# lucasjinreal/yolov7_d2

Measured on AMD Instinct MI355X. Metric: images/sec training, YOLOX-s 640x640 bs=16/GPU, higher is better.
Workload: dtype bf16; 1 GPU; YOLOX-s CSPDarknet+PAFPN 640x640 bs=16/GPU: fwd + SimOTA loss + bwd + grad all-reduce + SGD(momentum) step, uint8 image batch + labels resident in HBM; global_batch=16, parallelism=dp1, hipgraph=True

## Files before the change

### yolov7_d2_amd/csrc/conv3x3_ws.h

```cpp
#pragma once
#include "common.h"
#include "conv_bn.h"

#define W3_MAX_JOBS 8
#define W3_TW 16
template <int S, int TH>
struct W3Geo {
  static constexpr int HH = S == 1 ? TH + 2 : 2 * TH + 1;
  static constexpr int HW = S == 1 ? W3_TW + 2 : 2 * W3_TW + 1;
  static constexpr int HPIX = HH * HW;
  static constexpr int HROWS = (HPIX + 63) / 64 * 64;
  static constexpr int tap(int dy, int dx) { return S == 1 ? dy * HW + dx : dy * HW + (dx & 1) * (W3_TW + 1) + (dx >> 1); }
};

struct W3Job {
  const __bf16* x;
  const u32x4* w;
  __bf16* y;
  double* stats;
  int ldx, ldy, N, H, W, tilesY, tilesX, ntiles;
  int blk0, nblk;
  int wld, nslots, sld, pad_;
  int tw[9];
  int inH;
  int inW, xfw;
  const BnXf* xf;
};
struct W3K {
  int njobs, dbg;
  W3Job j[W3_MAX_JOBS];
};
struct W3Launch {
  int K, MODE, grid, lds, S, XF;
  W3K k;
};

#define W3_VMCNT(n) asm volatile("s_waitcnt vmcnt(%0)" ::"n"(n) : "memory")

static __device__ uint4 g_w3_zero_page[4];

__device__ __forceinline__ void w3_glds16(const void* g, unsigned lds_off) {
  asm volatile("s_mov_b32 m0, %1\n\ts_nop 0\n\tglobal_load_lds_dwordx4 %0, off" ::"v"(g), "s"(lds_off) : "memory");
}

template <int K, int WM, int WN, int G, int MODE, int S = 1, int TH = 8, int XF = 0>
__global__ __launch_bounds__(WM* WN * 64, (K == 128 || (S == 2 && K == 64)) ? 1 : 2) void w3_kernel(const W3K p) {
  static_assert(!XF || MODE == 1, "the input transform comes with the forward (statistics) mode");
  constexpr int NW = WM * WN, KC8 = K / 8, KS = K / 16;
  using Geo = W3Geo<S, TH>;
  constexpr int W3_TH = TH, W3_HW = Geo::HW, W3_HPIX = Geo::HPIX, W3_HROWS = Geo::HROWS;
  static_assert(WN * G * 32 == W3_TH * W3_TW, "pixel tile");
  constexpr int PLANE = W3_HROWS * 16;
  constexpr int NQ = (W3_HROWS / 64) * KC8;
  constexpr int D = NQ / NW;
  static_assert(NQ % NW == 0 && D >= 1, "DMA split");
  constexpr int XB = KC8 * PLANE;
  static_assert((KC8 - 1) * PLANE + Geo::tap(2, 2) * 16 < 65536, "ds_read immediate");
  constexpr int NS = 9 * KS, NTS = NS / 3;
  constexpr int NST = 2 * G;
  constexpr int DST = 2 * (D - 1) < NTS ? 2 : 1, SST = 2 * NST + NST / 2 <= NTS ? 2 : 1;
  static_assert(DST * (D - 1) < NTS && SST * NST + (MODE == 2 ? NST / 2 : 0) <= NTS, "the memory operations of a tile fit its main loop");

  extern __shared__ __attribute__((aligned(16))) char smem[];
  const unsigned lds0 = (unsigned)(uintptr_t)(__attribute__((address_space(3))) char*)smem;
  const int tid = threadIdx.x, lane = tid & 63;
  const int wave = __builtin_amdgcn_readfirstlane(tid >> 6);
  const int wm = wave / WN, wn = wave % WN;
  const int l31 = lane & 31, h = lane >> 5;

  int ji = 0;
  while (ji + 1 < p.njobs && (int)blockIdx.x >= p.j[ji + 1].blk0) ++ji;
  ji = __builtin_amdgcn_readfirstlane(ji);
  const W3Job& jb = p.j[ji];
  const int b = (int)blockIdx.x - jb.blk0, nb = jb.nblk;
  const int nt = (jb.ntiles - b + nb - 1) / nb;
  constexpr bool STATS = MODE == 1;
  const int H = jb.H, Wd = jb.W, tilesX = jb.tilesX, tpi = jb.tilesY * jb.tilesX;
  const int inH = S == 1 ? jb.H : jb.inH, inW = S == 1 ? jb.W : jb.inW;
  const int ldxb = jb.ldx * 2, ldyb = jb.ldy * 2;
  const char* const xbase = (const char*)jb.x;
  char* const ybase = (char*)jb.y;
  const char* zpage = (const char*)g_w3_zero_page;
  asm volatile("" : "+s"(zpage));
  float* const s_sc = (float*)(smem + 2 * (K / 8) * Geo::HROWS * 16 + 256 * 32 * 4);
  float* const s_sh = s_sc + K;
  int xf_act = 0, xf_ldab = 0;
  char* xf_a = nullptr;
  if constexpr (XF) {
    const BnXf* const xf = jb.xf;
    bnx_tables(xf, s_sc, s_sh, NW * 64, jb.xfw != 0 && b == 0);
    xf_act = xf->bn.act;
    xf_ldab = xf->bn.lda * 2;
    xf_a = jb.xfw ? (char*)xf->bn.a : nullptr;
  }

  bf16x8 a[9][KS];
  {
    const u32x4* wb = jb.w + wm * 32 + l31;
#pragma unroll
    for (int t = 0; t < 9; ++t) {
      const int slab = jb.tw[t] * KC8;
#pragma unroll
      for (int ks = 0; ks < KS; ++ks) a[t][ks] = __builtin_bit_cast(bf16x8, wb[(size_t)(slab + ks * 2 + h) * jb.wld]);
    }
  }

  struct Org { int img, ty0, tx0; };
  auto tile_origin = [&](int i) {
    const int t = b + i * nb;
    Org o;
    o.img = t / tpi;
    const int rem = t - o.img * tpi, tyq = rem / tilesX;
    o.ty0 = tyq * W3_TH;
    o.tx0 = (rem - tyq * tilesX) * W3_TW;
    return o;
  };
  auto issue_x1 = [&](const Org& o, int buf, int d) {
    const int iy0 = S * o.ty0 - 1, ix0 = S * o.tx0 - 1;
    const char* xt = xbase + ((size_t)o.img * inH * inW + (ptrdiff_t)iy0 * inW + ix0) * (ptrdiff_t)ldxb;
    const int q = wave * D + d;
    const int pb = q / KC8, k8 = q % KC8;
    const int pix = pb * 64 + lane;
    const int hy = S == 1 ? (int)(((unsigned)pix * 3641u) >> 16) : (int)(((unsigned)pix * 1986u) >> 16);
    const int hp = pix - hy * W3_HW;
    const int hx = S == 1 ? hp : (hp <= W3_TW ? 2 * hp : 2 * (hp - (W3_TW + 1)) + 1);
    const bool v = (pix < W3_HPIX) & ((unsigned)(iy0 + hy) < (unsigned)inH) & ((unsigned)(ix0 + hx) < (unsigned)inW);
    const char* g = v ? xt + (unsigned)((hy * inW + hx) * ldxb + k8 * 16) : zpage;
    w3_glds16(g, lds0 + buf * XB + k8 * PLANE + pb * 1024);
  };

  int lg, lidx;
  {
    const int l = l31;
    lg = ((l >= 4) & (l < 12)) | ((l >= 16) & (l < 20)) | (l >= 28);
    lidx = l - (l < 4 ? 0 : l < 12 ? 4 : l < 20 ? 8 : l < 28 ? 12 : 16);
  }
  unsigned bbase[G];
#pragma unroll
  for (int g = 0; g < G; ++g) bbase[g] = (unsigned)(h * PLANE + (S * ((wn * G + g) * 2 + lg) * W3_HW + lidx) * 16);
  auto out_ptr = [&](const Org& o, int g) -> char* {
    const int py = o.ty0 + (wn * G + g) * 2 + lg, px = o.tx0 + lidx;
    char* q = ybase + (((size_t)o.img * H + py) * Wd + px) * (size_t)ldyb + wm * 64 + h * 16;
    return ((py < H) & (px < Wd)) ? q : nullptr;
  };

  constexpr bool SREG = (K == 32 && S == 1) || (K == 64 && S == 2);
  float* const sacc = (float*)(smem + 2 * XB) + tid * 4;
  constexpr int SAS = NW * 64 * 4;
  float s1[16], s2[16];
  if constexpr (STATS) {
    if constexpr (SREG) {
#pragma unroll
      for (int r = 0; r < 16; ++r) s1[r] = s2[r] = 0.f;
    } else {
#pragma unroll
      for (int q = 0; q < 8; ++q) *(f32x4*)(sacc + q * SAS) = f32x4{0.f, 0.f, 0.f, 0.f};
    }
  }

  Org oc = tile_origin(0), op = oc;
#pragma unroll
  for (int d = 0; d < D; ++d) issue_x1(oc, 0, d);

  u32x4 pk[NST];
#pragma unroll
  for (int q = 0; q < NST; ++q) pk[q] = u32x4{0u, 0u, 0u, 0u};
  for (int i = 0; i < nt; ++i) {
    W3_VMCNT(0);
    if constexpr (XF) {
      if (i == 0) __syncthreads();
      const int iy0 = S * oc.ty0 - 1, ix0 = S * oc.tx0 - 1;
      char* const Xw = smem + (i & 1) * XB;
      char* const at = xf_a + ((size_t)oc.img * inH * inW + (ptrdiff_t)iy0 * inW + ix0) * (ptrdiff_t)xf_ldab;
#pragma unroll 2
      for (int d = 0; d < D; ++d) {
        const int q = wave * D + d;
        const int pb = q / KC8, k8 = q % KC8;
        const int pix = pb * 64 + lane;
        const int hy = S == 1 ? (int)(((unsigned)pix * 3641u) >> 16) : (int)(((unsigned)pix * 1986u) >> 16);
        const int hp = pix - hy * W3_HW;
        const int hx = S == 1 ? hp : (hp <= W3_TW ? 2 * hp : 2 * (hp - (W3_TW + 1)) + 1);
        const bool v = (pix < W3_HPIX) & ((unsigned)(iy0 + hy) < (unsigned)inH) & ((unsigned)(ix0 + hx) < (unsigned)inW);
        const u32x4 o = bnx_apply_lds(Xw + k8 * PLANE + pb * 1024 + lane * 16, s_sc, s_sh, k8, xf_act, v);
        const bool inner = v & (hy >= 1) & (hy <= S * W3_TH) & (hx >= 1) & (hx <= S * W3_TW);
        if (xf_a && inner) *(u32x4*)(at + (unsigned)((hy * inW + hx) * xf_ldab + k8 * 16)) = o;
      }
      asm volatile("s_waitcnt lgkmcnt(0)" ::: "memory");
    }
    __builtin_amdgcn_s_barrier();
    const bool more = (i + 1 < nt) & !(p.dbg & 2);
    const bool prev = i > 0;
    const Org on = tile_origin(i + 1 < nt ? i + 1 : i);
    const char* Xs = smem + (i & 1) * XB;
    u32x4 old[NST];

    f32x16 acc[G];
#pragma unroll
    for (int g = 0; g < G; ++g)
#pragma unroll
      for (int r = 0; r < 16; ++r) acc[g][r] = 0.f;
    auto ldb = [&](int step, bf16x8(&dst)[G]) {
      const int t9 = step / KS, ks = step % KS, dy = t9 / 3, dx = t9 % 3;
#pragma unroll
      for (int g = 0; g < G; ++g)
        dst[g] = __builtin_bit_cast(bf16x8, *(const u32x4*)(Xs + bbase[g] + (2 * ks * PLANE + Geo::tap(dy, dx) * 16)));
    };
    bf16x8 bf[3][G];
    ldb(0, bf[0]);
    ldb(1, bf[1]);
    if (!(p.dbg & 4))
#pragma unroll
    for (int ts = 0; ts < NTS; ++ts) {
      if (ts % DST == 0 && ts / DST < D) {
        if (more) issue_x1(on, (i + 1) & 1, ts / DST);
      }
      if (ts % SST == SST - 1 && ts / SST < NST) {
        char* q = prev ? out_ptr(op, (ts / SST) / 2) : nullptr;
        if (q) *(u32x4*)(q + ((ts / SST) % 2) * 32) = pk[ts / SST];
      }
      if constexpr (MODE == 2) {
        if (ts >= SST * NST && ts < SST * NST + NST / 2) {
#pragma unroll
          for (int l = 2 * (ts - SST * NST); l < 2 * (ts - SST * NST) + 2; ++l) {
            char* q = out_ptr(oc, l / 2);
            old[l] = u32x4{0u, 0u, 0u, 0u};
            if (q) {
              if (l % 2 == 0) asm volatile("global_load_dwordx4 %0, %1, off" : "+v"(old[l]) : "v"(q) : "memory");
              else asm volatile("global_load_dwordx4 %0, %1, off offset:32" : "+v"(old[l]) : "v"(q) : "memory");
            }
          }
        }
      }
#pragma unroll
      for (int r = 0; r < 3; ++r) {
        const int st = 3 * ts + r;
        __builtin_amdgcn_sched_barrier(0);
        if (st + 2 < NS) ldb(st + 2, bf[(r + 2) % 3]);
#pragma unroll
        for (int g = 0; g < G; ++g)
          acc[g] = __builtin_amdgcn_mfma_f32_32x32x16_bf16(a[st / KS][st % KS], bf[r][g], acc[g], 0, 0, 0);
#pragma unroll
        for (int g = 0; g < G; ++g) {
          __builtin_amdgcn_sched_group_barrier(0x008, 1, 0);
          __builtin_amdgcn_sched_group_barrier(0x100, 1, 0);
          __builtin_amdgcn_sched_group_barrier(0x002, 2, 0);
        }
      }
      __builtin_amdgcn_sched_barrier(0);
    }

    if constexpr (MODE == 2) {
      if constexpr (NST == 2)
        asm volatile("s_waitcnt vmcnt(0)" : "+v"(old[0]), "+v"(old[1])::"memory");
      else if constexpr (NST == 4)
        asm volatile("s_waitcnt vmcnt(0)" : "+v"(old[0]), "+v"(old[1]), "+v"(old[2]), "+v"(old[3])::"memory");
      else
        asm volatile("s_waitcnt vmcnt(0)"
                     : "+v"(old[0]), "+v"(old[1]), "+v"(old[2]), "+v"(old[3]), "+v"(old[4]), "+v"(old[5]), "+v"(old[6]), "+v"(old[7])::"memory");
    }
    if constexpr (STATS && !SREG) {
#pragma unroll
      for (int q = 0; q < 4; ++q) {
        const f32x4 u = *(const f32x4*)(sacc + q * SAS), w = *(const f32x4*)(sacc + (4 + q) * SAS);
#pragma unroll
        for (int e = 0; e < 4; ++e) { s1[4 * q + e] = u[e]; s2[4 * q + e] = w[e]; }
      }
    }
#pragma unroll
    for (int g = 0; g < G; ++g) {
      bool pvg = true;
      if constexpr (STATS) pvg = out_ptr(oc, g) != nullptr;
      unsigned pw[8];
#pragma unroll
      for (int q = 0; q < 4; ++q) {
        bf16x4 o;
#pragma unroll
        for (int e = 0; e < 4; ++e) o[e] = (__bf16)acc[g][4 * q + e];
        if constexpr (STATS) {
#pragma unroll
          for (int e = 0; e < 4; ++e) {
            const float f = pvg ? (float)o[e] : 0.f;
            s1[4 * q + e] += f;
            s2[4 * q + e] = __builtin_fmaf(f, f, s2[4 * q + e]);
          }
        }
        const u32x2 u = __builtin_bit_cast(u32x2, o);
        pw[2 * q] = u[0];
        pw[2 * q + 1] = u[1];
      }
#pragma unroll
      for (int pr = 0; pr < 2; ++pr) {
        const int q0 = 2 * pr, q1 = 2 * pr + 1;
        const auto w0 = __builtin_amdgcn_permlane32_swap(pw[2 * q0], pw[2 * q1], false, false);
        const auto w1 = __builtin_amdgcn_permlane32_swap(pw[2 * q0 + 1], pw[2 * q1 + 1], false, false);
        u32x4 v = {w0[0], w1[0], w0[1], w1[1]};
        if constexpr (MODE == 2) {
          const bf16x8 nv = __builtin_bit_cast(bf16x8, v), ov = __builtin_bit_cast(bf16x8, old[g * 2 + pr]);
          bf16x8 rv;
#pragma unroll
          for (int e = 0; e < 8; ++e) rv[e] = (__bf16)((float)nv[e] + (float)ov[e]);
          v = __builtin_bit_cast(u32x4, rv);
        }
        pk[g * 2 + pr] = v;
      }
    }
    if constexpr (STATS && !SREG) {
#pragma unroll
      for (int q = 0; q < 4; ++q) {
        *(f32x4*)(sacc + q * SAS) = f32x4{s1[4 * q], s1[4 * q + 1], s1[4 * q + 2], s1[4 * q + 3]};
        *(f32x4*)(sacc + (4 + q) * SAS) = f32x4{s2[4 * q], s2[4 * q + 1], s2[4 * q + 2], s2[4 * q + 3]};
      }
    }
    op = oc;
    oc = on;
  }
#pragma unroll
  for (int q = 0; q < NST; ++q) {
    char* o = out_ptr(op, q / 2);
    if (o) *(u32x4*)(o + (q % 2) * 32) = pk[q];
  }

  if constexpr (STATS) {
    if constexpr (!SREG) {
#pragma unroll
      for (int q = 0; q < 4; ++q) {
        const f32x4 u = *(const f32x4*)(sacc + q * SAS), w = *(const f32x4*)(sacc + (4 + q) * SAS);
#pragma unroll
        for (int e = 0; e < 4; ++e) { s1[4 * q + e] = u[e]; s2[4 * q + e] = w[e]; }
      }
    }
    cbn_block_stats<WM, WN>(s1, s2, (float*)smem, wave, lane, (p.dbg & 1) != 0, [&](const int c) {
      return jb.stats + (size_t)((int)blockIdx.x % jb.nslots) * jb.sld + c * 2;
    });
  }
}

template <int K, int WM, int WN, int G, int MODE, int S = 1, int TH = 8, int XF = 0>
static int w3_launch_one(const W3Launch& l, hipStream_t s) {
  auto fn = w3_kernel<K, WM, WN, G, MODE, S, TH, XF>;
  static bool attr_done = false;
  if (!attr_done) {
    hipFuncSetAttribute((const void*)fn, hipFuncAttributeMaxDynamicSharedMemorySize, 160 * 1024);
    attr_done = true;
  }
  hipLaunchKernelGGL(fn, dim3((unsigned)l.grid), dim3(WM * WN * 64), (size_t)l.lds, s, l.k);
  MI_CHECK_LAUNCH("conv3x3_ws");
  return MI_OK;
}
constexpr int w3_tile_h(int S, int K) { return S == 1 ? 8 : (K == 128 ? 2 : 4); }
constexpr int w3_block_cout(int S, int K) { return S == 1 ? K : (K == 32 ? 64 : 128); }
template <int MODE, int XF = 0>
static int w3_launch_mode(const W3Launch& l, hipStream_t s) {
  if (l.S == 2) {
    if constexpr (MODE == 1 || MODE == 0) {
      switch (l.K) {
        case 128: return w3_launch_one<128, 4, 1, 1, MODE, 2, 2, XF>(l, s);
        case 64: return w3_launch_one<64, 4, 1, 2, MODE, 2, 4, XF>(l, s);
        case 32: return w3_launch_one<32, 2, 2, 1, MODE, 2, 4, XF>(l, s);
      }
    }
    MI_FAIL(MI_EINVAL, "conv3x3_ws: stride 2 with K %d / mode %d", l.K, MODE);
  }
  switch (l.K) {
    case 128: return w3_launch_one<128, 4, 1, 4, MODE, 1, 8, XF>(l, s);
    case 64: return w3_launch_one<64, 2, 2, 2, MODE, 1, 8, XF>(l, s);
    case 32: return w3_launch_one<32, 1, 4, 1, MODE, 1, 8, XF>(l, s);
  }
  MI_FAIL(MI_EINVAL, "conv3x3_ws: K %d", l.K);
}
```

### yolov7_d2_amd/csrc/conv3x3_ws.hip

```cpp
#include <stdlib.h>
#include <string.h>
#include "common.h"
#include "conv3x3_ws.h"

int w3_launch_mode0(const W3Launch& l, hipStream_t s);
int w3_launch_mode1(const W3Launch& l, hipStream_t s);
int w3_launch_mode1x(const W3Launch& l, hipStream_t s);
int w3_launch_mode2(const W3Launch& l, hipStream_t s);

static int w3_cus() {
  static int cus = 0;
  if (!cus) {
    int dev = 0;
    hipDeviceProp_t pr;
    if (hipGetDevice(&dev) == hipSuccess && hipGetDeviceProperties(&pr, dev) == hipSuccess) cus = pr.multiProcessorCount;
    if (cus <= 0) cus = 256;
  }
  return cus;
}

static bool w3_desc_ok(const mi_conv_desc* d, int* tw) {
  const int K = d->K8 * 8;
  if (d->ntaps != 9 || (d->in_stride != 1 && d->in_stride != 2) || d->out_stride != 1 || d->out_oy || d->out_ox) return false;
  if (d->gridH != d->outH || d->gridW != d->outW) return false;
  if (d->flags & ~MI_CONV_ACCUM) return false;
  if (d->bias) return false;
  if (!(K == 32 || K == 64 || K == 128) || d->Cout != d->CoutPad) return false;
  if (d->in_stride == 1) {
    if (d->outH != d->H || d->outW != d->W || d->Cout != K) return false;
  } else {
    const char* s2 = getenv("MI_CONV_WS_S2");
    if ((s2 && atoi(s2) == 0) || (d->flags & MI_CONV_ACCUM)) return false;
    if (d->outH != (d->H - 1) / 2 + 1 || d->outW != (d->W - 1) / 2 + 1) return false;
    const int bc = w3_block_cout(2, K);
    if (d->Cout % bc || d->Cout / bc > W3_MAX_JOBS) return false;
  }
  if (d->ldx % 8 || d->ldy % 8 || ((uintptr_t)d->x & 15) || ((uintptr_t)d->y & 15) || ((uintptr_t)d->w & 15)) return false;
  if (d->y_nstride && (long long)d->y_nstride != (long long)d->outH * d->outW * d->ldy) return false;
  if ((long long)d->H * d->W * d->ldx * 2 >= (1LL << 31)) return false;
  if ((d->flags & MI_CONV_ACCUM) && d->stats_acc) return false;
  int seen = 0;
  for (int t = 0; t < 9; ++t) {
    const int dy = d->tap_dy[t], dx = d->tap_dx[t];
    if (dy < -1 || dy > 1 || dx < -1 || dx > 1) return false;
    const int pos = (dy + 1) * 3 + dx + 1;
    if (seen & (1 << pos)) return false;
    seen |= 1 << pos;
    tw[pos] = d->tap_w[t];
  }
  return seen == 0x1ff;
}

static bool w3_fill(const mi_conv_desc* ds, int n, W3Launch* l) {
  if (n < 1 || n > W3_MAX_JOBS) return false;
  memset(l, 0, sizeof(*l));
  const int K = ds[0].K8 * 8, S = ds[0].in_stride;
  const int mode = (ds[0].flags & MI_CONV_ACCUM) ? 2 : (ds[0].stats_acc ? 1 : 0);
  const bool xf = ds[0].xf != nullptr;
  if (xf && mode != 1) return false;
  const int TH = w3_tile_h(S, K);
  const int hrows = ((S == 1 ? (TH + 2) * (W3_TW + 2) : (2 * TH + 1) * (2 * W3_TW + 1)) + 63) / 64 * 64;
  const int lds = 2 * (K / 8) * hrows * 16 + (mode == 1 ? 256 * 32 * 4 : 0) + (xf ? 2 * K * 4 : 0);
  long long total = 0;
  int nj = 0;
  for (int j = 0; j < n; ++j) {
    const mi_conv_desc& d = ds[j];
    int tw[9];
    if (!w3_desc_ok(&d, tw) || d.K8 * 8 != K || d.in_stride != S) return false;
    if ((d.flags & MI_CONV_ACCUM) != (ds[0].flags & MI_CONV_ACCUM) || (d.stats_acc != nullptr) != (ds[0].stats_acc != nullptr)) return false;
    if ((d.xf != nullptr) != xf || (xf && (d.xf_C != K || ((uintptr_t)d.xf & 7)))) return false;
    const int bc = w3_block_cout(S, K);
    for (int c0 = 0; c0 < d.Cout; c0 += bc, ++nj) {
      if (nj >= W3_MAX_JOBS) return false;
      W3Job& jb = l->k.j[nj];
      memcpy(jb.tw, tw, sizeof(tw));
      jb.x = (const __bf16*)d.x; jb.w = (const u32x4*)d.w + c0; jb.y = (__bf16*)d.y + c0;
      jb.stats = d.stats_acc ? d.stats_acc + (size_t)c0 * 2 : nullptr;
      jb.ldx = d.ldx; jb.ldy = d.ldy; jb.N = d.N; jb.H = d.outH; jb.W = d.outW; jb.inH = d.H; jb.inW = d.W;
      jb.tilesY = mi_cdiv(d.outH, TH); jb.tilesX = mi_cdiv(d.outW, W3_TW);
      jb.ntiles = d.N * jb.tilesY * jb.tilesX;
      jb.wld = d.CoutPad;
      jb.nslots = (d.stats_slots >= 1 && d.stats_slots <= MI_BN_SLOTS) ? d.stats_slots : MI_BN_SLOTS;
      jb.sld = d.CoutPad * 2;
      total += jb.ntiles;
      jb.xf = (const BnXf*)d.xf;
      jb.xfw = (xf && d.xf_write && c0 == 0) ? 1 : 0;
    }
  }
  n = nj;
  int per_cu = K == 128 ? 1 : (K == 64 ? 2 : 4);
  if (S == 2) per_cu = (160 * 1024) / lds >= 2 && K != 128 ? 2 : 1;
  long long cap = (long long)w3_cus() * per_cu;
  if (cap > total) cap = total;
  int used = 0;
  for (int j = 0; j < n; ++j) {
    W3Job& jb = l->k.j[j];
    long long nb = (cap * jb.ntiles) / total;
    if (nb < 1) nb = 1;
    if (nb > jb.ntiles) nb = jb.ntiles;
    jb.nblk = (int)nb;
    used += jb.nblk;
  }
  while (used < cap) {
    int best = -1;
    double br = 0;
    for (int j = 0; j < n; ++j) {
      const W3Job& jb = l->k.j[j];
      const double r = (double)jb.ntiles / jb.nblk;
      if (jb.nblk < jb.ntiles && r > br) { br = r; best = j; }
    }
    if (best < 0) break;
    l->k.j[best].nblk++;
    used++;
  }
  int blk = 0;
  for (int j = 0; j < n; ++j) {
    l->k.j[j].blk0 = blk;
    blk += l->k.j[j].nblk;
  }
  l->k.njobs = n;
  l->k.dbg = (getenv("MI_DEBUG_NOATOM") ? atoi(getenv("MI_DEBUG_NOATOM")) & 1 : 0) | (getenv("MI_W3_DBG") ? atoi(getenv("MI_W3_DBG")) & 6 : 0);
  l->K = K;
  l->S = S;
  l->MODE = mode;
  l->XF = xf ? 1 : 0;
  l->grid = blk;
  l->lds = lds;
  return true;
}

static int w3_run(const W3Launch& l, hipStream_t s) {
  switch (l.MODE) {
    case 0: return w3_launch_mode0(l, s);
    case 1: return l.XF ? w3_launch_mode1x(l, s) : w3_launch_mode1(l, s);
    default: return w3_launch_mode2(l, s);
  }
}

static bool w3_enabled() {
  const char* e = getenv("MI_CONV_WS");
  return !e || atoi(e) != 0;
}

bool w3_try_launch(const mi_conv_desc* ds, int n, hipStream_t s, int* rc) {
  if (!w3_enabled()) return false;
  W3Launch l;
  if (!w3_fill(ds, n, &l)) return false;
  *rc = w3_run(l, s);
  return true;
}
bool w3_try_plan(const mi_conv_desc* ds, int n, W3Launch* l) { return w3_enabled() && w3_fill(ds, n, l); }
int w3_run_planned(const W3Launch* l, hipStream_t s) { return w3_run(*l, s); }

extern "C" int mi_conv3x3_ws(const mi_conv_desc* descs, int n, mi_stream_t st) {
  MI_REQUIRE(descs && n >= 1, "conv3x3_ws: null");
  W3Launch l;
  MI_REQUIRE(w3_fill(descs, n, &l),
             "conv3x3_ws: needs 1..%d bf16 3x3 stride-1 convs with K == Cout in {32, 64, 128} (all the same K), no bias, "
             "all plain / all with stats_acc / all MI_CONV_ACCUM", W3_MAX_JOBS);
  return w3_run(l, (hipStream_t)st);
}
```

Measured before the change: 3179 images/sec.

## Use buffer-resource loads/stores with OOB masking and incremental tile stepping in 3x3 conv

Replaces global_load_lds with zero-page redirection by buffer_load ... lds, using a buffer resource whose out-of-range offsets return zero. Output stores and MODE-2 reloads also go through raw buffer ops with an out-of-bounds sentinel instead of per-store pointer checks. Per-tile index math is reduced by precomputing halo pixel offsets once and advancing tile coordinates incrementally instead of dividing on every tile. It also adds an optional compile-time timeline probe and a new guard that output size fits in 31 bits.

```diff
diff --git a/yolov7_d2_amd/csrc/conv3x3_ws.h b/yolov7_d2_amd/csrc/conv3x3_ws.h
--- a/yolov7_d2_amd/csrc/conv3x3_ws.h
+++ b/yolov7_d2_amd/csrc/conv3x3_ws.h
@@ -29,6 +29,9 @@
 struct W3K {
   int njobs, dbg;
   W3Job j[W3_MAX_JOBS];
+#ifdef MI_W3_TIMELINE
+  unsigned long long* tl;
+#endif
 };
 struct W3Launch {
   int K, MODE, grid, lds, S, XF;
@@ -37,11 +40,43 @@
 
 #define W3_VMCNT(n) asm volatile("s_waitcnt vmcnt(%0)" ::"n"(n) : "memory")
 
-static __device__ uint4 g_w3_zero_page[4];
-
-__device__ __forceinline__ void w3_glds16(const void* g, unsigned lds_off) {
-  asm volatile("s_mov_b32 m0, %1\n\ts_nop 0\n\tglobal_load_lds_dwordx4 %0, off" ::"v"(g), "s"(lds_off) : "memory");
-}
+#define W3_OOB 0x80000000u
+
+__device__ __forceinline__ __amdgpu_buffer_rsrc_t w3_rsrc(const char* base, unsigned bytes) {
+  return __builtin_amdgcn_make_buffer_rsrc((void*)base, 0, (int)bytes, 0x00020000);
+}
+__device__ __forceinline__ void w3_blds16(__amdgpu_buffer_rsrc_t r, unsigned voff, unsigned soff, unsigned lds_off) {
+  asm volatile("s_mov_b32 m0, %3\n\ts_nop 3\n\tbuffer_load_dwordx4 %0, %1, %2 offen lds" ::"v"(voff), "s"(r), "s"(soff), "s"(lds_off) : "memory");
+}
+
+constexpr int w3_dma_blocks(int D, int KC8, int NW) {
+  int m = 1;
+  for (int w = 0; w < NW; ++w) {
+    const int n = (w * D + D - 1) / KC8 - (w * D) / KC8 + 1;
+    m = n > m ? n : m;
+  }
+  return m;
+}
+
+#ifdef MI_W3_TIMELINE
+#define W3_TL_POINTS 12
+#define W3_TL_BLOCKS 1024
+#define W3_TL(k)                                                                                              \
+  do {                                                                                                        \
+    __builtin_amdgcn_sched_barrier(0);                                                                        \
+    if (wave == 0 && blockIdx.x < W3_TL_BLOCKS) {                                                             \
+      unsigned long long tr_, tc_;                                                                            \
+      asm volatile("s_memrealtime %0\n\ts_memtime %1\n\ts_waitcnt lgkmcnt(0)" : "=s"(tr_), "=s"(tc_)::"memory"); \
+      if (lane == 0) {                                                                                        \
+        p.tl[((size_t)blockIdx.x * W3_TL_POINTS + (k)) * 2] = tr_;                                            \
+        p.tl[((size_t)blockIdx.x * W3_TL_POINTS + (k)) * 2 + 1] = tc_;                                        \
+      }                                                                                                       \
+    }                                                                                                         \
+    __builtin_amdgcn_sched_barrier(0);                                                                        \
+  } while (0)
+#else
+#define W3_TL(k) do { } while (0)
+#endif
 
 template <int K, int WM, int WN, int G, int MODE, int S = 1, int TH = 8, int XF = 0>
 __global__ __launch_bounds__(WM* WN * 64, (K == 128 || (S == 2 && K == 64)) ? 1 : 2) void w3_kernel(const W3K p) {
@@ -75,13 +110,13 @@
   const int b = (int)blockIdx.x - jb.blk0, nb = jb.nblk;
   const int nt = (jb.ntiles - b + nb - 1) / nb;
   constexpr bool STATS = MODE == 1;
-  const int H = jb.H, Wd = jb.W, tilesX = jb.tilesX, tpi = jb.tilesY * jb.tilesX;
+  const int H = jb.H, Wd = jb.W, tilesX = jb.tilesX, tilesY = jb.tilesY, tpi = jb.tilesY * jb.tilesX;
   const int inH = S == 1 ? jb.H : jb.inH, inW = S == 1 ? jb.W : jb.inW;
   const int ldxb = jb.ldx * 2, ldyb = jb.ldy * 2;
   const char* const xbase = (const char*)jb.x;
   char* const ybase = (char*)jb.y;
-  const char* zpage = (const char*)g_w3_zero_page;
-  asm volatile("" : "+s"(zpage));
+  const unsigned imgxb = (unsigned)(inH * inW * ldxb), imgyb = (unsigned)(H * Wd * ldyb);
+  W3_TL(0);
   float* const s_sc = (float*)(smem + 2 * (K / 8) * Geo::HROWS * 16 + 256 * 32 * 4);
   float* const s_sh = s_sc + K;
   int xf_act = 0, xf_ldab = 0;
@@ -105,28 +140,63 @@
     }
   }
 
-  struct Org { int img, ty0, tx0; };
-  auto tile_origin = [&](int i) {
-    const int t = b + i * nb;
-    Org o;
-    o.img = t / tpi;
-    const int rem = t - o.img * tpi, tyq = rem / tilesX;
-    o.ty0 = tyq * W3_TH;
-    o.tx0 = (rem - tyq * tilesX) * W3_TW;
+  struct Org { int img, ty, tx; };
+  int s_img, s_ty, s_tx;
+  Org oc;
+  {
+    s_img = nb / tpi;
+    const int r1 = nb - s_img * tpi;
+    s_ty = r1 / tilesX;
+    s_tx = r1 - s_ty * tilesX;
+    oc.img = b / tpi;
+    const int r0 = b - oc.img * tpi;
+    oc.ty = r0 / tilesX;
+    oc.tx = r0 - oc.ty * tilesX;
+  }
+  auto tile_next = [&](Org o) {
+    o.tx += s_tx;
+    const int cx = o.tx >= tilesX;
+    o.tx -= cx ? tilesX : 0;
+    o.ty += s_ty + cx;
+    const int cy = o.ty >= tilesY;
+    o.ty -= cy ? tilesY : 0;
+    o.img += s_img + cy;
     return o;
   };
-  auto issue_x1 = [&](const Org& o, int buf, int d) {
-    const int iy0 = S * o.ty0 - 1, ix0 = S * o.tx0 - 1;
-    const char* xt = xbase + ((size_t)o.img * inH * inW + (ptrdiff_t)iy0 * inW + ix0) * (ptrdiff_t)ldxb;
-    const int q = wave * D + d;
-    const int pb = q / KC8, k8 = q % KC8;
-    const int pix = pb * 64 + lane;
+  constexpr int NPB = w3_dma_blocks(D, KC8, NW);
+  static_assert(NPB <= 2, "sel");
+  const int pb0 = (wave * D) / KC8;
+  unsigned hpix[NPB], hoff[NPB];
+#pragma unroll
+  for (int j = 0; j < NPB; ++j) {
+    const int pix = (pb0 + j) * 64 + lane;
     const int hy = S == 1 ? (int)(((unsigned)pix * 3641u) >> 16) : (int)(((unsigned)pix * 1986u) >> 16);
     const int hp = pix - hy * W3_HW;
     const int hx = S == 1 ? hp : (hp <= W3_TW ? 2 * hp : 2 * (hp - (W3_TW + 1)) + 1);
-    const bool v = (pix < W3_HPIX) & ((unsigned)(iy0 + hy) < (unsigned)inH) & ((unsigned)(ix0 + hx) < (unsigned)inW);
-    const char* g = v ? xt + (unsigned)((hy * inW + hx) * ldxb + k8 * 16) : zpage;
-    w3_glds16(g, lds0 + buf * XB + k8 * PLANE + pb * 1024);
+    const bool in = pix < W3_HPIX;
+    hpix[j] = in ? (unsigned)(hy << 8 | hx) : 0u;
+    hoff[j] = in ? (unsigned)((hy * inW + hx) * ldxb) : W3_OOB;
+  }
+  auto sel = [&](const unsigned(&a)[NPB], int j) {
+    return NPB > 1 && j >= 1 ? a[NPB - 1] : a[0];
+  };
+  struct XT { const char* img; unsigned v[NPB]; };
+  auto x_tile = [&](const Org& o) {
+    const int iy0 = S * o.ty * W3_TH - 1, ix0 = S * o.tx * W3_TW - 1;
+    const unsigned tb = (unsigned)((iy0 * inW + ix0) * ldxb);
+    XT t;
+    t.img = xbase + (size_t)o.img * imgxb;
+#pragma unroll
+    for (int j = 0; j < NPB; ++j) {
+      const bool v = ((unsigned)(iy0 + (int)(hpix[j] >> 8)) < (unsigned)inH) & ((unsigned)(ix0 + (int)(hpix[j] & 255u)) < (unsigned)inW);
+      t.v[j] = v ? tb + hoff[j] : W3_OOB;
+    }
+    return t;
+  };
+  auto issue_x1 = [&](const XT& t, int buf, int d) {
+    const int q = wave * D + d;
+    const int pb = q / KC8, k8 = q % KC8;
+    w3_blds16(w3_rsrc(t.img, imgxb), sel(t.v, pb - pb0), (unsigned)(k8 * 16), lds0 + buf * XB + k8 * PLANE + pb * 1024);
   };
 
   int lg, lidx;
@@ -138,11 +208,18 @@
   unsigned bbase[G];
 #pragma unroll
   for (int g = 0; g < G; ++g) bbase[g] = (unsigned)(h * PLANE + (S * ((wn * G + g) * 2 + lg) * W3_HW + lidx) * 16);
-  auto out_ptr = [&](const Org& o, int g) -> char* {
-    const int py = o.ty0 + (wn * G + g) * 2 + lg, px = o.tx0 + lidx;
-    char* q = ybase + (((size_t)o.img * H + py) * Wd + px) * (size_t)ldyb + wm * 64 + h * 16;
-    return ((py < H) & (px < Wd)) ? q : nullptr;
+  const unsigned yoff0 = (unsigned)((((wn * G) * 2 + lg) * Wd + lidx) * ldyb + wm * 64 + h * 16), ystep = (unsigned)(2 * Wd * ldyb);
+  struct YT { char* img; unsigned v; int rows; };
+  auto y_tile = [&](const Org& o) {
+    const int ty0 = o.ty * W3_TH, tx0 = o.tx * W3_TW;
+    YT t;
+    t.img = ybase + (size_t)o.img * imgyb;
+    t.v = lidx < Wd - tx0 ? (unsigned)((ty0 * Wd + tx0) * ldyb) + yoff0 : W3_OOB;
+    t.rows = H - ty0 - wn * G * 2;
+    return t;
   };
+  auto y_valid = [&](const YT& t, int g) { return (lg < t.rows - 2 * g) & (t.v != W3_OOB); };
+  auto y_off = [&](const YT& t, int g) { return lg < t.rows - 2 * g ? t.v + g * ystep : W3_OOB; };
 
   constexpr bool SREG = (K == 32 && S == 1) || (K == 64 && S == 2);
   float* const sacc = (float*)(smem + 2 * XB) + tid * 4;
@@ -158,9 +235,17 @@
     }
   }
 
-  Org oc = tile_origin(0), op = oc;
-#pragma unroll
-  for (int d = 0; d < D; ++d) issue_x1(oc, 0, d);
+#ifdef MI_W3_TIMELINE
+  W3_VMCNT(0);
+#endif
+  W3_TL(1);
+  {
+    const XT x0 = x_tile(oc);
+#pragma unroll
+    for (int d = 0; d < D; ++d) issue_x1(x0, 0, d);
+  }
+  YT yc = y_tile(oc), yp = yc;
+  yp.v = W3_OOB;
 
   u32x4 pk[NST];
 #pragma unroll
@@ -169,18 +254,16 @@
     W3_VMCNT(0);
     if constexpr (XF) {
       if (i == 0) __syncthreads();
-      const int iy0 = S * oc.ty0 - 1, ix0 = S * oc.tx0 - 1;
+      const int iy0 = S * oc.ty * W3_TH - 1, ix0 = S * oc.tx * W3_TW - 1;
       char* const Xw = smem + (i & 1) * XB;
       char* const at = xf_a + ((size_t)oc.img * inH * inW + (ptrdiff_t)iy0 * inW + ix0) * (ptrdiff_t)xf_ldab;
 #pragma unroll 2
       for (int d = 0; d < D; ++d) {
         const int q = wave * D + d;
         const int pb = q / KC8, k8 = q % KC8;
-        const int pix = pb * 64 + lane;
-        const int hy = S == 1 ? (int)(((unsigned)pix * 3641u) >> 16) : (int)(((unsigned)pix * 1986u) >> 16);
-        const int hp = pix - hy * W3_HW;
-        const int hx = S == 1 ? hp : (hp <= W3_TW ? 2 * hp : 2 * (hp - (W3_TW + 1)) + 1);
-        const bool v = (pix < W3_HPIX) & ((unsigned)(iy0 + hy) < (unsigned)inH) & ((unsigned)(ix0 + hx) < (unsigned)inW);
+        const unsigned hp = sel(hpix, pb - pb0);
+        const int hy = (int)(hp >> 8), hx = (int)(hp & 255u);
+        const bool v = (sel(hoff, pb - pb0) != W3_OOB) & ((unsigned)(iy0 + hy) < (unsigned)inH) & ((unsigned)(ix0 + hx) < (unsigned)inW);
         const u32x4 o = bnx_apply_lds(Xw + k8 * PLANE + pb * 1024 + lane * 16, s_sc, s_sh, k8, xf_act, v);
         const bool inner = v & (hy >= 1) & (hy <= S * W3_TH) & (hx >= 1) & (hx <= S * W3_TW);
         if (xf_a && inner) *(u32x4*)(at + (unsigned)((hy * inW + hx) * xf_ldab + k8 * 16)) = o;
@@ -188,9 +271,13 @@
       asm volatile("s_waitcnt lgkmcnt(0)" ::: "memory");
     }
     __builtin_amdgcn_s_barrier();
+#ifdef MI_W3_TIMELINE
+    if (i == 0) W3_TL(2);
+    if (i < 3) W3_TL(3 + 2 * i);
+#endif
     const bool more = (i + 1 < nt) & !(p.dbg & 2);
-    const bool prev = i > 0;
-    const Org on = tile_origin(i + 1 < nt ? i + 1 : i);
+    const Org on = tile_next(oc);
+    const XT xn = x_tile(on);
     const char* Xs = smem + (i & 1) * XB;
     u32x4 old[NST];
 
@@ -212,23 +299,17 @@
 #pragma unroll
     for (int ts = 0; ts < NTS; ++ts) {
       if (ts % DST == 0 && ts / DST < D) {
-        if (more) issue_x1(on, (i + 1) & 1, ts / DST);
-      }
-      if (ts % SST == SST - 1 && ts / SST < NST) {
-        char* q = prev ? out_ptr(op, (ts / SST) / 2) : nullptr;
-        if (q) *(u32x4*)(q + ((ts / SST) % 2) * 32) = pk[ts / SST];
-      }
+        if (more) issue_x1(xn, (i + 1) & 1, ts / DST);
+      }
+      if (ts % SST == SST - 1 && ts / SST < NST)
+        __builtin_amdgcn_raw_buffer_store_b128(pk[ts / SST], w3_rsrc(yp.img, imgyb), y_off(yp, (ts / SST) / 2) + ((ts / SST) % 2) * 32, 0, 0);
       if constexpr (MODE == 2) {
         if (ts >= SST * NST && ts < SST * NST + NST / 2) {
-#pragma unroll
-          for (int l = 2 * (ts - SST * NST); l < 2 * (ts - SST * NST) + 2; ++l) {
-            char* q = out_ptr(oc, l / 2);
-            old[l] = u32x4{0u, 0u, 0u, 0u};
-            if (q) {
-              if (l % 2 == 0) asm volatile("global_load_dwordx4 %0, %1, off" : "+v"(old[l]) : "v"(q) : "memory");
-              else asm volatile("global_load_dwordx4 %0, %1, off offset:32" : "+v"(old[l]) : "v"(q) : "memory");
-            }
-          }
+          const int l = 2 * (ts - SST * NST);
+          const unsigned vo = y_off(yc, l / 2);
+          const __amdgpu_buffer_rsrc_t yr = w3_rsrc(yc.img, imgyb);
+          asm volatile("buffer_load_dwordx4 %0, %1, %2, 0 offen" : "=v"(old[l]) : "v"(vo), "s"(yr) : "memory");
+          asm volatile("buffer_load_dwordx4 %0, %1, %2, 0 offen offset:32" : "=v"(old[l + 1]) : "v"(vo), "s"(yr) : "memory");
         }
       }
 #pragma unroll
@@ -248,6 +329,9 @@
       }
       __builtin_amdgcn_sched_barrier(0);
     }
+#ifdef MI_W3_TIMELINE
+    if (i < 3) W3_TL(4 + 2 * i);
+#endif
 
     if constexpr (MODE == 2) {
       if constexpr (NST == 2)
@@ -269,7 +353,7 @@
 #pragma unroll
     for (int g = 0; g < G; ++g) {
       bool pvg = true;
-      if constexpr (STATS) pvg = out_ptr(oc, g) != nullptr;
+      if constexpr (STATS) pvg = y_valid(yc, g);
       unsigned pw[8];
 #pragma unroll
       for (int q = 0; q < 4; ++q) {
@@ -311,14 +395,14 @@
         *(f32x4*)(sacc + (4 + q) * SAS) = f32x4{s2[4 * q], s2[4 * q + 1], s2[4 * q + 2], s2[4 * q + 3]};
       }
     }
-    op = oc;
     oc = on;
-  }
-#pragma unroll
-  for (int q = 0; q < NST; ++q) {
-    char* o = out_ptr(op, q / 2);
-    if (o) *(u32x4*)(o + (q % 2) * 32) = pk[q];
-  }
+    yp = yc;
+    yc = y_tile(oc);
+  }
+#pragma unroll
+  for (int q = 0; q < NST; ++q)
+    __builtin_amdgcn_raw_buffer_store_b128(pk[q], w3_rsrc(yp.img, imgyb), y_off(yp, q / 2) + (q % 2) * 32, 0, 0);
+  W3_TL(9);
 
   if constexpr (STATS) {
     if constexpr (!SREG) {
@@ -333,6 +417,11 @@
       return jb.stats + (size_t)((int)blockIdx.x % jb.nslots) * jb.sld + c * 2;
     });
   }
+  W3_TL(10);
+#ifdef MI_W3_TIMELINE
+  W3_VMCNT(0);
+#endif
+  W3_TL(11);
 }
 
 template <int K, int WM, int WN, int G, int MODE, int S = 1, int TH = 8, int XF = 0>
diff --git a/yolov7_d2_amd/csrc/conv3x3_ws.hip b/yolov7_d2_amd/csrc/conv3x3_ws.hip
--- a/yolov7_d2_amd/csrc/conv3x3_ws.hip
+++ b/yolov7_d2_amd/csrc/conv3x3_ws.hip
@@ -7,6 +7,19 @@
 int w3_launch_mode1(const W3Launch& l, hipStream_t s);
 int w3_launch_mode1x(const W3Launch& l, hipStream_t s);
 int w3_launch_mode2(const W3Launch& l, hipStream_t s);
+
+#ifdef MI_W3_TIMELINE
+static unsigned long long* w3_tl_buf() {
+  static unsigned long long* buf = nullptr;
+  if (!buf && (hipMalloc((void**)&buf, W3_TL_BLOCKS * W3_TL_POINTS * 16) != hipSuccess || hipMemset(buf, 0, W3_TL_BLOCKS * W3_TL_POINTS * 16) != hipSuccess)) buf = nullptr;
+  return buf;
+}
+extern "C" int mi_debug_w3_timeline(unsigned long long* host) {
+  unsigned long long* buf = w3_tl_buf();
+  if (!buf || hipMemcpy(host, buf, W3_TL_BLOCKS * W3_TL_POINTS * 16, hipMemcpyDeviceToHost) != hipSuccess) return -1;
+  return hipMemset(buf, 0, W3_TL_BLOCKS * W3_TL_POINTS * 16) == hipSuccess ? 0 : -1;
+}
+#endif
 
 static int w3_cus() {
   static int cus = 0;
@@ -38,6 +51,7 @@
   if (d->ldx % 8 || d->ldy % 8 || ((uintptr_t)d->x & 15) || ((uintptr_t)d->y & 15) || ((uintptr_t)d->w & 15)) return false;
   if (d->y_nstride && (long long)d->y_nstride != (long long)d->outH * d->outW * d->ldy) return false;
   if ((long long)d->H * d->W * d->ldx * 2 >= (1LL << 31)) return false;
+  if ((long long)d->outH * d->outW * d->ldy * 2 >= (1LL << 31) || (long long)d->outW * d->ldy * 2 * 8 >= (1LL << 31)) return false;
   if ((d->flags & MI_CONV_ACCUM) && d->stats_acc) return false;
   int seen = 0;
   for (int t = 0; t < 9; ++t) {
@@ -120,6 +134,10 @@
   }
   l->k.njobs = n;
   l->k.dbg = (getenv("MI_DEBUG_NOATOM") ? atoi(getenv("MI_DEBUG_NOATOM")) & 1 : 0) | (getenv("MI_W3_DBG") ? atoi(getenv("MI_W3_DBG")) & 6 : 0);
+#ifdef MI_W3_TIMELINE
+  l->k.tl = w3_tl_buf();
+  if (!l->k.tl) return false;
+#endif
   l->K = K;
   l->S = S;
   l->MODE = mode;
```

After: 3193 images/sec, median of 6. About the same (+0.4%).
